# geoeo/ORB_SLAM3_V1.0

Measured on AMD Instinct MI355X. Metric: frames/sec ORB extract+match, 752x480 8-level 1000-feat; bit-exact kp/desc, higher is better.
Workload: dtype u8

## Files before the change

### orb_slam3_v1.0_amd/csrc/fast_common.h

```cpp
#pragma once
#include <hip/hip_runtime.h>
#include <stdint.h>

namespace orbfe {

constexpr int kFastTW = 64, kFastTH = 32;

constexpr int kFusedPyramidMinFrames = 0;

__device__ __forceinline__ bool arc9(uint32_t m)
{
    uint32_t m2 = m | (m << 16);
    uint32_t r = m2 & (m2 >> 1);
    r &= r >> 2;
    r &= r >> 4;
    r &= m2 >> 8;
    return (r & 0xffffu) != 0;
}

__device__ __forceinline__ bool corner_at_global(const uint8_t* __restrict__ img, int pitch, int x, int y, int th)
{
    const int8_t dy[16] = {3, 3, 2, 1, 0, -1, -2, -3, -3, -3, -2, -1, 0, 1, 2, 3};
    const int8_t dx[16] = {0, 1, 2, 3, 3, 3, 2, 1, 0, -1, -2, -3, -3, -3, -2, -1};
    const int v = img[(size_t)y * pitch + x];
    uint32_t mb = 0, md = 0;
#pragma unroll
    for (int k = 0; k < 16; k++) {
        const int d = (int)img[(size_t)(y + dy[k]) * pitch + x + dx[k]] - v;
        mb |= (uint32_t)(d > th) << k;
        md |= (uint32_t)(d < -th) << k;
    }
    return arc9(mb) || arc9(md);
}

}
```

### orb_slam3_v1.0_amd/csrc/kernels_quadtree.hip

```cpp
#include "launch.h"
#include "fast_common.h"

namespace orbfe {

constexpr int kQtThreads = 512;
constexpr int kQtThreadsSmall = 1024;
constexpr int kQtMaxRounds = 48;
constexpr uint32_t kKeyInf = 0x01000000u;

struct Box {
    int16_t ulx, urx, uly, bry;
};

__device__ __forceinline__ int child_code(const Box& b, int x, int y)
{
    const int halfX = (b.urx - b.ulx + 1) >> 1;
    const int halfY = (b.bry - b.uly + 1) >> 1;
    const int right = !(x < b.ulx + halfX);
    const int bottom = !(y < b.uly + halfY);
    return right + 2 * bottom;
}

__device__ __forceinline__ Box child_box(const Box& b, int c)
{
    const int halfX = (b.urx - b.ulx + 1) >> 1;
    const int halfY = (b.bry - b.uly + 1) >> 1;
    Box r;
    r.ulx = (c & 1) ? (int16_t)(b.ulx + halfX) : b.ulx;
    r.urx = (c & 1) ? b.urx : (int16_t)(b.ulx + halfX);
    r.uly = (c & 2) ? (int16_t)(b.uly + halfY) : b.uly;
    r.bry = (c & 2) ? b.bry : (int16_t)(b.uly + halfY);
    return r;
}

template <int NT>
__device__ __forceinline__ int block_excl_scan(int v, int& total, int* sWave)
{
    const int lane = threadIdx.x & 63, wave = threadIdx.x >> 6;
    int incl = v;
    incl += __builtin_amdgcn_update_dpp(0, incl, 0x111, 0xF, 0xF, true);
    incl += __builtin_amdgcn_update_dpp(0, incl, 0x112, 0xF, 0xF, true);
    incl += __builtin_amdgcn_update_dpp(0, incl, 0x114, 0xF, 0xF, true);
    incl += __builtin_amdgcn_update_dpp(0, incl, 0x118, 0xF, 0xF, true);
    incl += __builtin_amdgcn_update_dpp(0, incl, 0x142, 0xA, 0xF, true);
    incl += __builtin_amdgcn_update_dpp(0, incl, 0x143, 0xC, 0xF, true);
    __syncthreads();
    if (lane == 63) sWave[wave] = incl;
    __syncthreads();
    int base = 0, tot = 0;
#pragma unroll
    for (int i = 0; i < NT / 64; i++) {
        const int s = sWave[i];
        if (i < wave) base += s;
        tot += s;
    }
    total = tot;
    return base + incl - v;
}

template <int NT>
__device__ uint32_t pre_nms_cut_key(const PipelineDesc* __restrict__ P, const LevelDesc& L, int f, int l, bool high,
                                    int nFast, const uint8_t* __restrict__ gray0, size_t gray0FrameStride, int gray0Pitch,
                                    const uint8_t* __restrict__ ws, const uint16_t* __restrict__ tileRows, int* sWave,
                                    int* sRed)
{
    const int tid = threadIdx.x;
    const uint16_t* tr = tileRows + ((size_t)f * P->totalTiles + L.tileBase) * kFastTH;
    if (tid == 0) { sRed[0] = -1; sRed[1] = 0; sRed[2] = -1; }
    __syncthreads();
    int carry = 0;
    for (int base = 0; base < L.h; base += NT) {
        const int y = base + tid;
        int c = 0;
        if (y < L.h) {
            const int ty = y / kFastTH, r = y % kFastTH;
            for (int tx = 0; tx < L.tilesX; tx++) {
                const uint32_t v = tr[(size_t)(ty * L.tilesX + tx) * kFastTH + r];
                c += high ? (int)(v >> 8) : (int)(v & 0xffu);
            }
        }
        int tot;
        const int ex = block_excl_scan<NT>(c, tot, sWave) + carry;
        if (c > 0 && ex < nFast && ex + c >= nFast) { sRed[0] = y; sRed[1] = nFast - ex; }
        carry += tot;
        __syncthreads();
        if (sRed[0] >= 0) break;
    }
    const int ys = sRed[0], q = sRed[1];
    if (ys < 0) return kKeyInf;
    const uint8_t* img;
    int pitch;
    if (l == 0) {
        img = gray0 + (size_t)f * gray0FrameStride;
        pitch = gray0Pitch;
    } else {
        img = ws + L.imgOff + (size_t)f * L.imgFrameStride;
        pitch = L.pitch;
    }
    const int th = high ? P->iniTh : P->minTh;
    carry = 0;
    for (int base = 0; base < L.w; base += NT) {
        const int x = base + tid;
        int flag = 0;
        if (x > kEdge && x < L.w - kEdge) flag = corner_at_global(img, pitch, x, ys, th) ? 1 : 0;
        int tot;
        const int ex = block_excl_scan<NT>(flag, tot, sWave) + carry;
        if (flag && ex + 1 == q) sRed[2] = x;
        carry += tot;
        __syncthreads();
        if (sRed[2] >= 0) break;
    }
    const int xs = sRed[2];
    __syncthreads();
    if (xs < 0) return kKeyInf;
    return (((uint32_t)ys << kCoordBits) | (uint32_t)xs) + 1u;
}

__host__ __device__ constexpr size_t qt_scratch_bytes(int nc) { return (size_t)nc * (8 + 8 + 8 + 4 + 4 + 16 + 4 + 4 + 4 + 1 + 1); }

template <int NC, bool GLOBAL, int NT = kQtThreads>
__global__ __launch_bounds__(NT) __attribute__((amdgpu_waves_per_eu(NC <= 512 ? 8 : 1))) void quadtree_kernel(const PipelineDesc* __restrict__ P,
                                                             const uint32_t* __restrict__ cand,
                                                             uint16_t* __restrict__ nodeOfAll,
                                                             uint32_t* __restrict__ counters,
                                                             uint32_t* __restrict__ lvlKp,
                                                             const uint8_t* __restrict__ gray0, size_t gray0FrameStride,
                                                             int gray0Pitch, const uint8_t* __restrict__ ws,
                                                             const uint16_t* __restrict__ tileRows,
                                                             uint8_t* __restrict__ scratch)
{
    constexpr int IPT = NC / NT;
    static_assert(NC % NT == 0, "NC must be a multiple of the block size");

    Box* sBox[2];
    int* sCnt[2];
    int* sCC;
    int* sKeep;
    int* sS;
    uint8_t* sSplit;
    uint8_t* sNch;
    unsigned long long* sKey;
    int* sProc;
    if constexpr (!GLOBAL) {
        __shared__ Box lBox[2][NC];
        __shared__ int lCnt[2][NC];
        __shared__ int lCC[NC * 4];
        __shared__ int lKeep[NC];
        __shared__ int lS[NC];
        __shared__ uint8_t lSplit[NC];
        __shared__ uint8_t lNch[NC];
        __shared__ unsigned long long lKey[NC];
        __shared__ int lProc[NC];
        sBox[0] = lBox[0]; sBox[1] = lBox[1]; sCnt[0] = lCnt[0]; sCnt[1] = lCnt[1];
        sCC = lCC; sKeep = lKeep; sS = lS; sSplit = lSplit; sNch = lNch; sKey = lKey; sProc = lProc;
    } else {
        uint8_t* base = scratch + ((size_t)blockIdx.y * gridDim.x + blockIdx.x) * qt_scratch_bytes(NC);
        sKey = reinterpret_cast<unsigned long long*>(base); base += (size_t)NC * 8;
        sBox[0] = reinterpret_cast<Box*>(base); base += (size_t)NC * 8;
        sBox[1] = reinterpret_cast<Box*>(base); base += (size_t)NC * 8;
        sCnt[0] = reinterpret_cast<int*>(base); base += (size_t)NC * 4;
        sCnt[1] = reinterpret_cast<int*>(base); base += (size_t)NC * 4;
        sCC = reinterpret_cast<int*>(base); base += (size_t)NC * 16;
        sKeep = reinterpret_cast<int*>(base); base += (size_t)NC * 4;
        sS = reinterpret_cast<int*>(base); base += (size_t)NC * 4;
        sProc = reinterpret_cast<int*>(base); base += (size_t)NC * 4;
        sSplit = base; base += NC;
        sNch = base;
    }
    __shared__ int sWave[NT / 64];
    __shared__ int sRed[4];

    const int f = blockIdx.x, l = blockIdx.y;
    const int nL = P->nLevels;
    const LevelDesc& L = P->lv[l];
    const int tid = threadIdx.x;
    uint32_t* cnt = counters + ((size_t)f * nL + l) * kCntWords;
    const uint32_t* C = cand + L.candOff + (size_t)f * L.candCap;
    uint16_t* nodeOf = nodeOfAll + L.candOff + (size_t)f * L.candCap;
    uint32_t* out = lvlKp + (size_t)f * P->kpCapFrame + L.kpBase;

    const int N = L.nFeatures;
    const int nFast = P->nFast;
    const int iniTh = P->iniTh;
    const int nAll = (int)min(cnt[kCntCand], (uint32_t)L.candCap);
    uint32_t cutHi = kKeyInf, cutLo = kKeyInf;
    int cH = (int)cnt[kCntHigh];
    if ((int)cnt[kCntPreHigh] > nFast) {
        cutHi = pre_nms_cut_key<NT>(P, L, f, l, true, nFast, gray0, gray0FrameStride, gray0Pitch, ws, tileRows, sWave, sRed);
        int c = 0;
        for (int p = tid; p < nAll; p += NT) c += cand_score(C[p]) >= iniTh && cand_key(C[p]) < cutHi;
        block_excl_scan<NT>(c, cH, sWave);
    }
    const unsigned diff = (unsigned)nFast - (unsigned)cH;
    const bool retry = (double)diff > 0.25 * (double)nFast;
    int cL = nAll;
    if (retry && (int)cnt[kCntPreLow] > nFast) {
        cutLo = pre_nms_cut_key<NT>(P, L, f, l, false, nFast, gray0, gray0FrameStride, gray0Pitch, ws, tileRows, sWave, sRed);
        int c = 0;
        for (int p = tid; p < nAll; p += NT) c += cand_key(C[p]) < cutLo;
        block_excl_scan<NT>(c, cL, sWave);
    }
    uint32_t keyCut = cutLo;
    int lowKept = 0;
    if (retry && cL > 0) {
        lowKept = cL;
        if (cH + cL > nFast) lowKept = max(nFast - cH, 0);
    }
    if (retry && lowKept < cL) {
        uint32_t lo = 0, hi = kKeyInf;
        while (lo < hi) {
            const uint32_t mid = lo + ((hi - lo) >> 1);
            int c = 0;
            for (int p = tid; p < nAll; p += NT) c += cand_key(C[p]) < mid;
            int tot;
            block_excl_scan<NT>(c, tot, sWave);
            if (tot >= lowKept) hi = mid; else lo = mid + 1;
        }
        keyCut = min(lo, cutLo);
    }
    cL = nAll;
    const int totalPts = cH + lowKept;
    if (totalPts == 0) {
        if (tid == 0) cnt[kCntKp] = 0;
        return;
    }
    if (L.nodeCap > NC) {
        if (tid == 0) { cnt[kCntKp] = 0; atomicOr(&cnt[kCntStatus], (uint32_t)kFlagNodeOverflow); }
        return;
    }

#define PT_WEIGHT(cw) ((int)(cand_score(cw) >= iniTh && cand_key(cw) < cutHi) + (int)(retry && cand_key(cw) < keyCut))

    const int nIni = L.nIni;
    const float hX = L.hX;
    for (int i = tid; i < NC; i += NT) sCnt[0][i] = 0;
    __syncthreads();
    for (int p = tid; p < cL; p += NT) {
        const uint32_t cw = C[p];
        const int wgt = PT_WEIGHT(cw);
        if (wgt) atomicAdd(&sCnt[0][(int)((float)cand_x(cw) / hX)], wgt);
    }
    __syncthreads();
    if (tid == 0) {
        int n = 0;
        for (int i = 0; i < nIni; i++) {
            const int c = sCnt[0][i];
            sKeep[i] = n;
            if (c > 0) {
                Box b;
                b.ulx = (int16_t)(int)(hX * (float)i);
                b.urx = (int16_t)(int)(hX * (float)(i + 1));
                b.uly = 0;
                b.bry = (int16_t)L.h;
                sBox[1][n] = b;
                sCnt[1][n] = c;
                n++;
            }
        }
        sRed[0] = n;
    }
    __syncthreads();
    int n = sRed[0];
    for (int p = tid; p < cL; p += NT) {
        const uint32_t cw = C[p];
        if (PT_WEIGHT(cw)) nodeOf[p] = (uint16_t)sKeep[(int)((float)cand_x(cw) / hX)];
    }
    int cur = 1;
    bool sortedMode = false;
    bool overflow = false;

    for (int round = 0; round < kQtMaxRounds; round++) {
        const int prevSize = n;
        Box* box = cur ? sBox[1] : sBox[0];
        int* ncnt = cur ? sCnt[1] : sCnt[0];
        Box* nbox = cur ? sBox[0] : sBox[1];
        int* nncnt = cur ? sCnt[0] : sCnt[1];

        for (int i = tid; i < n * 4; i += NT) sCC[i] = 0;
        __syncthreads();
        for (int p0 = tid; p0 < cL; p0 += 4 * NT) {
            uint32_t cw4[4];
            int nd4[4];
#pragma unroll
            for (int k = 0; k < 4; k++) {
                const int p = p0 + k * NT;
                cw4[k] = p < cL ? C[p] : 0u;
                nd4[k] = p < cL ? (int)nodeOf[p] : 0;
            }
#pragma unroll
            for (int k = 0; k < 4; k++) {
                const uint32_t cw = cw4[k];
                const int wgt = (p0 + k * NT < cL) ? PT_WEIGHT(cw) : 0;
                if (wgt) {
                    const int i = nd4[k];
                    if (ncnt[i] > 1) atomicAdd(&sCC[4 * i + child_code(box[i], cand_x(cw), cand_y(cw))], wgt);
                }
            }
        }
        __syncthreads();

        int myExp[IPT], myNch[IPT];
#pragma unroll
        for (int k = 0; k < IPT; k++) {
            const int i = tid * IPT + k;
            int e = 0, nc = 0;
            if (i < n && ncnt[i] > 1) {
                e = 1;
                nc = (sCC[4 * i] > 0) + (sCC[4 * i + 1] > 0) + (sCC[4 * i + 2] > 0) + (sCC[4 * i + 3] > 0);
            }
            myExp[k] = e;
            myNch[k] = nc;
            if (i < NC) { sNch[i] = (uint8_t)nc; sSplit[i] = 0; }
        }

        int T = 0;
        if (!sortedMode) {
            int loc = 0;
#pragma unroll
            for (int k = 0; k < IPT; k++) loc += myNch[k];
            int base = block_excl_scan<NT>(loc, T, sWave);
#pragma unroll
            for (int k = 0; k < IPT; k++) {
                const int i = tid * IPT + k;
                if (i < n) {
                    sS[i] = base;
                    sSplit[i] = (uint8_t)myExp[k];
                }
                base += myNch[k];
            }
        } else {
#pragma unroll
            for (int k = 0; k < IPT; k++) {
                const int i = tid * IPT + k;
                if (i < n) {
                    unsigned long long key = 0;
                    if (myExp[k])
                        key = ((unsigned long long)(uint32_t)ncnt[i] << 40) |
                              ((unsigned long long)(uint16_t)box[i].ulx << 28) |
                              ((unsigned long long)(uint16_t)box[i].uly << 16) |
                              (unsigned long long)(0xFFFFu - (uint32_t)i);
                    sKey[i] = key;
                }
            }
            __syncthreads();
            int locM = 0;
#pragma unroll
            for (int k = 0; k < IPT; k++) locM += myExp[k];
            int m;
            block_excl_scan<NT>(locM, m, sWave);
#pragma unroll
            for (int k = 0; k < IPT; k++) {
                const int i = tid * IPT + k;
                if (i < n && myExp[k]) {
                    const unsigned long long key = sKey[i];
                    int r = 0;
                    for (int j = 0; j < n; j++) r += sKey[j] > key;
                    sProc[r] = i;
                }
            }
            __syncthreads();
            int locInc[IPT], locSum = 0;
#pragma unroll
            for (int k = 0; k < IPT; k++) {
                const int r = tid * IPT + k;
                locInc[k] = (r < m) ? (int)sNch[sProc[r]] - 1 : 0;
                locSum += locInc[k];
            }
            int totInc;
            int run = block_excl_scan<NT>(locSum, totInc, sWave);
            int myJ = m;
#pragma unroll
            for (int k = 0; k < IPT; k++) {
                const int r = tid * IPT + k;
                run += locInc[k];
                if (r < m && n + run >= N && myJ == m) myJ = r + 1;
            }
            if (tid == 0) sRed[1] = m;
            __syncthreads();
            if (myJ < m) atomicMin(&sRed[1], myJ);
            __syncthreads();
            const int J = sRed[1];
            int locN[IPT], locT = 0;
#pragma unroll
            for (int k = 0; k < IPT; k++) {
                const int r = tid * IPT + k;
                locN[k] = (r < J) ? (int)sNch[sProc[r]] : 0;
                locT += locN[k];
            }
            int base = block_excl_scan<NT>(locT, T, sWave);
#pragma unroll
            for (int k = 0; k < IPT; k++) {
                const int r = tid * IPT + k;
                if (r < J) {
                    const int i = sProc[r];
                    sS[i] = base;
                    sSplit[i] = 1;
                }
                base += locN[k];
            }
        }
        __syncthreads();

        int locK = 0;
#pragma unroll
        for (int k = 0; k < IPT; k++) {
            const int i = tid * IPT + k;
            locK += (i < n && !sSplit[i]) ? 1 : 0;
        }
        int K;
        int kbase = block_excl_scan<NT>(locK, K, sWave);
        const int newSize = T + K;
        if (newSize > NC) overflow = true;
        if (overflow) break;
        if (tid == 0) sRed[2] = 0;
        __syncthreads();

        int locExpand = 0;
#pragma unroll
        for (int k = 0; k < IPT; k++) {
            const int i = tid * IPT + k;
            if (i < n) {
                if (sSplit[i]) {
                    const Box b = box[i];
                    int kk = 0;
                    const int s = sS[i];
#pragma unroll
                    for (int c = 0; c < 4; c++) {
                        const int cc = sCC[4 * i + c];
                        if (cc > 0) {
                            const int pos = T - 1 - (s + kk);
                            nbox[pos] = child_box(b, c);
                            nncnt[pos] = cc;
                            sCC[4 * i + c] = pos;
                            locExpand += cc > 1;
                            kk++;
                        }
                    }
                } else {
                    const int pos = T + kbase;
                    nbox[pos] = box[i];
                    nncnt[pos] = ncnt[i];
                    sKeep[i] = pos;
                    kbase++;
                }
            }
        }
        if (locExpand) atomicAdd(&sRed[2], locExpand);
        __syncthreads();
        const int nToExpand = sRed[2];

        for (int p0 = tid; p0 < cL; p0 += 4 * NT) {
            uint32_t cw4[4];
            int nd4[4];
#pragma unroll
            for (int k = 0; k < 4; k++) {
                const int p = p0 + k * NT;
                cw4[k] = p < cL ? C[p] : 0u;
                nd4[k] = p < cL ? (int)nodeOf[p] : 0;
            }
#pragma unroll
            for (int k = 0; k < 4; k++) {
                const int p = p0 + k * NT;
                const uint32_t cw = cw4[k];
                if (p < cL && PT_WEIGHT(cw)) {
                    const int i = nd4[k];
                    nodeOf[p] = (uint16_t)(sSplit[i] ? sCC[4 * i + child_code(box[i], cand_x(cw), cand_y(cw))] : sKeep[i]);
                }
            }
        }
        __syncthreads();
        n = newSize;
        cur ^= 1;

        if (n >= N || n == prevSize) break;
        if (!sortedMode && n + 3 * nToExpand > N) sortedMode = true;
        if (round == kQtMaxRounds - 1 && tid == 0) atomicOr(&cnt[kCntStatus], (uint32_t)kFlagRoundLimit);
    }

    if (overflow) {
        if (tid == 0) { cnt[kCntKp] = 0; atomicOr(&cnt[kCntStatus], (uint32_t)kFlagNodeOverflow); }
        return;
    }

    int* bestResp = sCC;
    uint32_t* bestKey = reinterpret_cast<uint32_t*>(sCC + NC);
    for (int i = tid; i < n; i += NT) { bestResp[i] = 0; bestKey[i] = 0xFFFFFFFFu; }
    __syncthreads();
    for (int p = tid; p < cL; p += NT) {
        const uint32_t cw = C[p];
        if (PT_WEIGHT(cw)) atomicMax(&bestResp[nodeOf[p]], cand_score(cw));
    }
    __syncthreads();
    for (int p = tid; p < cL; p += NT) {
        const uint32_t cw = C[p];
        if (PT_WEIGHT(cw)) {
            const int i = nodeOf[p];
            if (cand_score(cw) == bestResp[i]) atomicMin(&bestKey[i], cand_key(cw));
        }
    }
    __syncthreads();
    for (int i = tid; i < n; i += NT) out[i] = ((uint32_t)bestResp[i] << 24) | bestKey[i];
    if (tid == 0) cnt[kCntKp] = (uint32_t)n;
#undef PT_WEIGHT
}

int quadtree_node_capacity(int maxNodeCap)
{
    const int caps[] = {512, 2048, 8192, 32768, 65536};
    for (int c : caps)
        if (maxNodeCap <= c && maxNodeCap <= 65535) return c;
    return 0;
}

size_t quadtree_scratch_bytes_per_block(int maxNodeCap)
{
    const int nc = quadtree_node_capacity(maxNodeCap);
    return nc > 2048 ? qt_scratch_bytes(nc) : 0;
}

void launch_quadtree(hipStream_t s, int frames, int nLevels, int maxNodeCap, const PipelineDesc* dP,
                     const uint32_t* cand, uint16_t* nodeOf, uint32_t* counters, uint32_t* lvlKp,
                     const uint8_t* gray0, size_t gray0FrameStride, int gray0Pitch, const uint8_t* ws,
                     const uint16_t* tileRows, uint8_t* scratch)
{
    dim3 grid(frames, nLevels);
    if ((long long)frames * nLevels <= 64 && quadtree_node_capacity(maxNodeCap) <= 2048) {
        dim3 blockS(kQtThreadsSmall);
        if (quadtree_node_capacity(maxNodeCap) <= 1024)
            hipLaunchKernelGGL((quadtree_kernel<1024, false, kQtThreadsSmall>), grid, blockS, 0, s, dP, cand, nodeOf, counters, lvlKp, gray0,
                               gray0FrameStride, gray0Pitch, ws, tileRows, scratch);
        else
            hipLaunchKernelGGL((quadtree_kernel<2048, false, kQtThreadsSmall>), grid, blockS, 0, s, dP, cand, nodeOf, counters, lvlKp, gray0,
                               gray0FrameStride, gray0Pitch, ws, tileRows, scratch);
        return;
    }
    dim3 block(kQtThreads);
#define ORBFE_QT(NCV, GLB)                                                                                        \
    hipLaunchKernelGGL((quadtree_kernel<NCV, GLB>), grid, block, 0, s, dP, cand, nodeOf, counters, lvlKp, gray0, \
                       gray0FrameStride, gray0Pitch, ws, tileRows, scratch)
    switch (quadtree_node_capacity(maxNodeCap)) {
    case 512: ORBFE_QT(512, false); break;
    case 2048: ORBFE_QT(2048, false); break;
    case 8192: ORBFE_QT(8192, true); break;
    case 32768: ORBFE_QT(32768, true); break;
    default: ORBFE_QT(65536, true); break;
    }
#undef ORBFE_QT
}

}
```

Measured before the change: 227,800.

## Keep quadtree candidates register-resident and fuse child counting into relabel pass

When a level has at most 4096 candidates and the kernel uses shared memory, the quadtree kernel now loads each candidate word and its node label into registers once and reuses them across every distribution round. The separate per-round child-count pass is folded into the previous round's relabel pass, which uses double-buffered child-count arrays so the global C/nodeOf reads drop out. Scans get double-buffered wave slots so a barrier can be dropped, two scans are fused into one, the sorted-mode rank loop runs only over compacted expandable keys with 16-byte loads, and the best-response selection becomes a single atomicMax on a packed key. This adds register pressure and doubles the child-count storage, which could lower occupancy.

```diff
diff --git a/orb_slam3_v1.0_amd/csrc/fast_common.h b/orb_slam3_v1.0_amd/csrc/fast_common.h
--- a/orb_slam3_v1.0_amd/csrc/fast_common.h
+++ b/orb_slam3_v1.0_amd/csrc/fast_common.h
@@ -7,6 +7,8 @@
 constexpr int kFastTW = 64, kFastTH = 32;
 
 constexpr int kFusedPyramidMinFrames = 0;
+
+constexpr int kQtResidentCap = 4096;
 
 __device__ __forceinline__ bool arc9(uint32_t m)
 {
diff --git a/orb_slam3_v1.0_amd/csrc/kernels_quadtree.hip b/orb_slam3_v1.0_amd/csrc/kernels_quadtree.hip
--- a/orb_slam3_v1.0_amd/csrc/kernels_quadtree.hip
+++ b/orb_slam3_v1.0_amd/csrc/kernels_quadtree.hip
@@ -33,10 +33,8 @@
     return r;
 }
 
-template <int NT>
-__device__ __forceinline__ int block_excl_scan(int v, int& total, int* sWave)
-{
-    const int lane = threadIdx.x & 63, wave = threadIdx.x >> 6;
+__device__ __forceinline__ int wave_incl_scan(int v)
+{
     int incl = v;
     incl += __builtin_amdgcn_update_dpp(0, incl, 0x111, 0xF, 0xF, true);
     incl += __builtin_amdgcn_update_dpp(0, incl, 0x112, 0xF, 0xF, true);
@@ -44,25 +42,62 @@
     incl += __builtin_amdgcn_update_dpp(0, incl, 0x118, 0xF, 0xF, true);
     incl += __builtin_amdgcn_update_dpp(0, incl, 0x142, 0xA, 0xF, true);
     incl += __builtin_amdgcn_update_dpp(0, incl, 0x143, 0xC, 0xF, true);
-    __syncthreads();
-    if (lane == 63) sWave[wave] = incl;
+    return incl;
+}
+
+template <int NT>
+__host__ __device__ constexpr int qt_wave_words() { return 2 * 2 * (NT / 64); }
+
+template <int NT>
+__device__ __forceinline__ int block_excl_scan(int v, int& total, int* sWave, int& par)
+{
+    constexpr int NW = NT / 64;
+    const int lane = threadIdx.x & 63, wave = threadIdx.x >> 6;
+    const int incl = wave_incl_scan(v);
+    int* w = sWave + par * 2 * NW;
+    par ^= 1;
+    if (lane == 63) w[wave] = incl;
     __syncthreads();
     int base = 0, tot = 0;
 #pragma unroll
-    for (int i = 0; i < NT / 64; i++) {
-        const int s = sWave[i];
+    for (int i = 0; i < NW; i++) {
+        const int s = w[i];
         if (i < wave) base += s;
         tot += s;
     }
-    total = tot;
+    total = __builtin_amdgcn_readfirstlane(tot);
     return base + incl - v;
+}
+
+template <int NT>
+__device__ __forceinline__ int block_excl_scan2(int a, int b, int& totA, int& totB, int& exB, int* sWave, int& par)
+{
+    constexpr int NW = NT / 64;
+    const int lane = threadIdx.x & 63, wave = threadIdx.x >> 6;
+    const int inA = wave_incl_scan(a), inB = wave_incl_scan(b);
+    int* w = sWave + par * 2 * NW;
+    par ^= 1;
+    if (lane == 63) { w[wave] = inA; w[NW + wave] = inB; }
+    __syncthreads();
+    int baseA = 0, tA = 0, baseB = 0, tB = 0;
+#pragma unroll
+    for (int i = 0; i < NW; i++) {
+        const int sa = w[i], sb = w[NW + i];
+        if (i < wave) { baseA += sa; baseB += sb; }
+        tA += sa;
+        tB += sb;
+    }
+    totA = __builtin_amdgcn_readfirstlane(tA);
+    totB = __builtin_amdgcn_readfirstlane(tB);
+    exB = baseB + inB - b;
+    return baseA + inA - a;
 }
 
 template <int NT>
 __device__ uint32_t pre_nms_cut_key(const PipelineDesc* __restrict__ P, const LevelDesc& L, int f, int l, bool high,
                                     int nFast, const uint8_t* __restrict__ gray0, size_t gray0FrameStride, int gray0Pitch,
                                     const uint8_t* __restrict__ ws, const uint16_t* __restrict__ tileRows, int* sWave,
-                                    int* sRed)
+                                    int& par, int* sRed)
 {
     const int tid = threadIdx.x;
     const uint16_t* tr = tileRows + ((size_t)f * P->totalTiles + L.tileBase) * kFastTH;
@@ -80,13 +115,13 @@
             }
         }
         int tot;
-        const int ex = block_excl_scan<NT>(c, tot, sWave) + carry;
+        const int ex = block_excl_scan<NT>(c, tot, sWave, par) + carry;
         if (c > 0 && ex < nFast && ex + c >= nFast) { sRed[0] = y; sRed[1] = nFast - ex; }
         carry += tot;
         __syncthreads();
         if (sRed[0] >= 0) break;
     }
-    const int ys = sRed[0], q = sRed[1];
+    const int ys = __builtin_amdgcn_readfirstlane(sRed[0]), q = __builtin_amdgcn_readfirstlane(sRed[1]);
     if (ys < 0) return kKeyInf;
     const uint8_t* img;
     int pitch;
@@ -104,19 +139,19 @@
         int flag = 0;
         if (x > kEdge && x < L.w - kEdge) flag = corner_at_global(img, pitch, x, ys, th) ? 1 : 0;
         int tot;
-        const int ex = block_excl_scan<NT>(flag, tot, sWave) + carry;
+        const int ex = block_excl_scan<NT>(flag, tot, sWave, par) + carry;
         if (flag && ex + 1 == q) sRed[2] = x;
         carry += tot;
         __syncthreads();
         if (sRed[2] >= 0) break;
     }
-    const int xs = sRed[2];
+    const int xs = __builtin_amdgcn_readfirstlane(sRed[2]);
     __syncthreads();
     if (xs < 0) return kKeyInf;
     return (((uint32_t)ys << kCoordBits) | (uint32_t)xs) + 1u;
 }
 
-__host__ __device__ constexpr size_t qt_scratch_bytes(int nc) { return (size_t)nc * (8 + 8 + 8 + 4 + 4 + 16 + 4 + 4 + 4 + 1 + 1); }
+__host__ __device__ constexpr size_t qt_scratch_bytes(int nc) { return (size_t)nc * (8 + 8 + 8 + 4 + 4 + 16 + 16 + 4 + 4 + 4 + 1 + 1); }
 
 template <int NC, bool GLOBAL, int NT = kQtThreads>
 __global__ __launch_bounds__(NT) __attribute__((amdgpu_waves_per_eu(NC <= 512 ? 8 : 1))) void quadtree_kernel(const PipelineDesc* __restrict__ P,
@@ -134,7 +169,7 @@
 
     Box* sBox[2];
     int* sCnt[2];
-    int* sCC;
+    int* sCCt[2];
     int* sKeep;
     int* sS;
     uint8_t* sSplit;
@@ -144,15 +179,15 @@
     if constexpr (!GLOBAL) {
         __shared__ Box lBox[2][NC];
         __shared__ int lCnt[2][NC];
-        __shared__ int lCC[NC * 4];
+        __shared__ __attribute__((aligned(16))) int lCC[2][NC * 4];
         __shared__ int lKeep[NC];
         __shared__ int lS[NC];
         __shared__ uint8_t lSplit[NC];
         __shared__ uint8_t lNch[NC];
-        __shared__ unsigned long long lKey[NC];
+        __shared__ __attribute__((aligned(16))) unsigned long long lKey[NC];
         __shared__ int lProc[NC];
         sBox[0] = lBox[0]; sBox[1] = lBox[1]; sCnt[0] = lCnt[0]; sCnt[1] = lCnt[1];
-        sCC = lCC; sKeep = lKeep; sS = lS; sSplit = lSplit; sNch = lNch; sKey = lKey; sProc = lProc;
+        sCCt[0] = lCC[0]; sCCt[1] = lCC[1]; sKeep = lKeep; sS = lS; sSplit = lSplit; sNch = lNch; sKey = lKey; sProc = lProc;
     } else {
         uint8_t* base = scratch + ((size_t)blockIdx.y * gridDim.x + blockIdx.x) * qt_scratch_bytes(NC);
         sKey = reinterpret_cast<unsigned long long*>(base); base += (size_t)NC * 8;
@@ -160,15 +195,17 @@
         sBox[1] = reinterpret_cast<Box*>(base); base += (size_t)NC * 8;
         sCnt[0] = reinterpret_cast<int*>(base); base += (size_t)NC * 4;
         sCnt[1] = reinterpret_cast<int*>(base); base += (size_t)NC * 4;
-        sCC = reinterpret_cast<int*>(base); base += (size_t)NC * 16;
+        sCCt[0] = reinterpret_cast<int*>(base); base += (size_t)NC * 16;
+        sCCt[1] = reinterpret_cast<int*>(base); base += (size_t)NC * 16;
         sKeep = reinterpret_cast<int*>(base); base += (size_t)NC * 4;
         sS = reinterpret_cast<int*>(base); base += (size_t)NC * 4;
         sProc = reinterpret_cast<int*>(base); base += (size_t)NC * 4;
         sSplit = base; base += NC;
         sNch = base;
     }
-    __shared__ int sWave[NT / 64];
+    __shared__ int sWave[qt_wave_words<NT>()];
     __shared__ int sRed[4];
+    int par = 0;
 
     const int f = blockIdx.x, l = blockIdx.y;
     const int nL = P->nLevels;
@@ -183,22 +220,34 @@
     const int nFast = P->nFast;
     const int iniTh = P->iniTh;
     const int nAll = (int)min(cnt[kCntCand], (uint32_t)L.candCap);
+    constexpr int KREG = GLOBAL ? 1 : kQtResidentCap / NT;
+    static_assert(GLOBAL || KREG * NT == kQtResidentCap, "the block size must divide kQtResidentCap");
+    const bool resident = !GLOBAL && nAll <= kQtResidentCap;
+    uint32_t rcw[KREG];
+    int rst[KREG];
+    if (resident) {
+#pragma unroll
+        for (int k = 0; k < KREG; k++) {
+            const int p = tid + k * NT;
+            rcw[k] = p < nAll ? C[p] : 0u;
+        }
+    }
     uint32_t cutHi = kKeyInf, cutLo = kKeyInf;
     int cH = (int)cnt[kCntHigh];
     if ((int)cnt[kCntPreHigh] > nFast) {
-        cutHi = pre_nms_cut_key<NT>(P, L, f, l, true, nFast, gray0, gray0FrameStride, gray0Pitch, ws, tileRows, sWave, sRed);
+        cutHi = pre_nms_cut_key<NT>(P, L, f, l, true, nFast, gray0, gray0FrameStride, gray0Pitch, ws, tileRows, sWave, par, sRed);
         int c = 0;
         for (int p = tid; p < nAll; p += NT) c += cand_score(C[p]) >= iniTh && cand_key(C[p]) < cutHi;
-        block_excl_scan<NT>(c, cH, sWave);
+        block_excl_scan<NT>(c, cH, sWave, par);
     }
     const unsigned diff = (unsigned)nFast - (unsigned)cH;
     const bool retry = (double)diff > 0.25 * (double)nFast;
     int cL = nAll;
     if (retry && (int)cnt[kCntPreLow] > nFast) {
-        cutLo = pre_nms_cut_key<NT>(P, L, f, l, false, nFast, gray0, gray0FrameStride, gray0Pitch, ws, tileRows, sWave, sRed);
+        cutLo = pre_nms_cut_key<NT>(P, L, f, l, false, nFast, gray0, gray0FrameStride, gray0Pitch, ws, tileRows, sWave, par, sRed);
         int c = 0;
         for (int p = tid; p < nAll; p += NT) c += cand_key(C[p]) < cutLo;
-        block_excl_scan<NT>(c, cL, sWave);
+        block_excl_scan<NT>(c, cL, sWave, par);
     }
     uint32_t keyCut = cutLo;
     int lowKept = 0;
@@ -213,7 +262,7 @@
             int c = 0;
             for (int p = tid; p < nAll; p += NT) c += cand_key(C[p]) < mid;
             int tot;
-            block_excl_scan<NT>(c, tot, sWave);
+            block_excl_scan<NT>(c, tot, sWave, par);
             if (tot >= lowKept) hi = mid; else lo = mid + 1;
         }
         keyCut = min(lo, cutLo);
@@ -231,15 +280,57 @@
 
 #define PT_WEIGHT(cw) ((int)(cand_score(cw) >= iniTh && cand_key(cw) < cutHi) + (int)(retry && cand_key(cw) < keyCut))
 
+    if (resident) {
+#pragma unroll
+        for (int k = 0; k < KREG; k++) rst[k] = (tid + k * NT < nAll) ? PT_WEIGHT(rcw[k]) << 16 : 0;
+    }
+    auto cand_pass = [&](auto readLabel, auto writeLabel, auto&& f) {
+        constexpr bool READ = decltype(readLabel)::value, WRITE = decltype(writeLabel)::value;
+        if (resident) {
+#pragma unroll
+            for (int k = 0; k < KREG; k++) {
+                const int st = rst[k], wgt = st >> 16;
+                asm volatile("" : "+v"(rcw[k]));
+                if (wgt) {
+                    const int lab = f(rcw[k], wgt, st & 0xFFFF);
+                    if constexpr (WRITE) rst[k] = (wgt << 16) | lab;
+                }
+            }
+            return;
+        }
+        for (int p0 = tid; p0 < cL; p0 += 4 * NT) {
+            uint32_t cw4[4];
+            int nd4[4];
+#pragma unroll
+            for (int k = 0; k < 4; k++) {
+                const int p = p0 + k * NT;
+                cw4[k] = p < cL ? C[p] : 0u;
+                nd4[k] = (READ && p < cL) ? (int)nodeOf[p] : 0;
+            }
+#pragma unroll
+            for (int k = 0; k < 4; k++) {
+                const int p = p0 + k * NT;
+                const uint32_t cw = cw4[k];
+                const int wgt = p < cL ? PT_WEIGHT(cw) : 0;
+                if (wgt) {
+                    const int lab = f(cw, wgt, nd4[k]);
+                    if constexpr (WRITE) nodeOf[p] = (uint16_t)lab;
+                }
+            }
+        }
+    };
+    constexpr std::true_type yes{};
+    constexpr std::false_type no{};
+
     const int nIni = L.nIni;
     const float hX = L.hX;
     for (int i = tid; i < NC; i += NT) sCnt[0][i] = 0;
-    __syncthreads();
-    for (int p = tid; p < cL; p += NT) {
-        const uint32_t cw = C[p];
-        const int wgt = PT_WEIGHT(cw);
-        if (wgt) atomicAdd(&sCnt[0][(int)((float)cand_x(cw) / hX)], wgt);
-    }
+    for (int i = tid; i < 4 * nIni; i += NT) sCCt[1][i] = 0;
+    __syncthreads();
+    cand_pass(no, no, [&](uint32_t cw, int wgt, int) {
+        atomicAdd(&sCnt[0][(int)((float)cand_x(cw) / hX)], wgt);
+        return 0;
+    });
     __syncthreads();
     if (tid == 0) {
         int n = 0;
@@ -260,11 +351,13 @@
         sRed[0] = n;
     }
     __syncthreads();
-    int n = sRed[0];
-    for (int p = tid; p < cL; p += NT) {
-        const uint32_t cw = C[p];
-        if (PT_WEIGHT(cw)) nodeOf[p] = (uint16_t)sKeep[(int)((float)cand_x(cw) / hX)];
-    }
+    int n = __builtin_amdgcn_readfirstlane(sRed[0]);
+    cand_pass(no, yes, [&](uint32_t cw, int wgt, int) {
+        const int i = sKeep[(int)((float)cand_x(cw) / hX)];
+        if (sCnt[1][i] > 1) atomicAdd(&sCCt[1][4 * i + child_code(sBox[1][i], cand_x(cw), cand_y(cw))], wgt);
+        return i;
+    });
+    __syncthreads();
     int cur = 1;
     bool sortedMode = false;
     bool overflow = false;
@@ -275,29 +368,10 @@
         int* ncnt = cur ? sCnt[1] : sCnt[0];
         Box* nbox = cur ? sBox[0] : sBox[1];
         int* nncnt = cur ? sCnt[0] : sCnt[1];
-
-        for (int i = tid; i < n * 4; i += NT) sCC[i] = 0;
-        __syncthreads();
-        for (int p0 = tid; p0 < cL; p0 += 4 * NT) {
-            uint32_t cw4[4];
-            int nd4[4];
-#pragma unroll
-            for (int k = 0; k < 4; k++) {
-                const int p = p0 + k * NT;
-                cw4[k] = p < cL ? C[p] : 0u;
-                nd4[k] = p < cL ? (int)nodeOf[p] : 0;
-            }
-#pragma unroll
-            for (int k = 0; k < 4; k++) {
-                const uint32_t cw = cw4[k];
-                const int wgt = (p0 + k * NT < cL) ? PT_WEIGHT(cw) : 0;
-                if (wgt) {
-                    const int i = nd4[k];
-                    if (ncnt[i] > 1) atomicAdd(&sCC[4 * i + child_code(box[i], cand_x(cw), cand_y(cw))], wgt);
-                }
-            }
-        }
-        __syncthreads();
+        int* sCC = cur ? sCCt[1] : sCCt[0];
+        int* nCC = cur ? sCCt[0] : sCCt[1];
+
+        if (tid == 0) sRed[2] = 0;
 
         int myExp[IPT], myNch[IPT];
 #pragma unroll
@@ -310,15 +384,18 @@
             }
             myExp[k] = e;
             myNch[k] = nc;
-            if (i < NC) { sNch[i] = (uint8_t)nc; sSplit[i] = 0; }
-        }
-
-        int T = 0;
+            if (i < NC) sNch[i] = (uint8_t)nc;
+        }
+
+        int T = 0, K = 0, kbase = 0;
         if (!sortedMode) {
-            int loc = 0;
-#pragma unroll
-            for (int k = 0; k < IPT; k++) loc += myNch[k];
-            int base = block_excl_scan<NT>(loc, T, sWave);
+            int locT = 0, locK = 0;
+#pragma unroll
+            for (int k = 0; k < IPT; k++) {
+                locT += myNch[k];
+                locK += (tid * IPT + k < n && !myExp[k]) ? 1 : 0;
+            }
+            int base = block_excl_scan2<NT>(locT, locK, T, K, kbase, sWave, par);
 #pragma unroll
             for (int k = 0; k < IPT; k++) {
                 const int i = tid * IPT + k;
@@ -329,33 +406,42 @@
                 base += myNch[k];
             }
         } else {
+            unsigned long long myKey[IPT];
+            int locM = 0;
 #pragma unroll
             for (int k = 0; k < IPT; k++) {
                 const int i = tid * IPT + k;
-                if (i < n) {
-                    unsigned long long key = 0;
-                    if (myExp[k])
-                        key = ((unsigned long long)(uint32_t)ncnt[i] << 40) |
-                              ((unsigned long long)(uint16_t)box[i].ulx << 28) |
-                              ((unsigned long long)(uint16_t)box[i].uly << 16) |
-                              (unsigned long long)(0xFFFFu - (uint32_t)i);
-                    sKey[i] = key;
-                }
+                myKey[k] = 0;
+                if (myExp[k])
+                    myKey[k] = ((unsigned long long)(uint32_t)ncnt[i] << 40) |
+                               ((unsigned long long)(uint16_t)box[i].ulx << 28) |
+                               ((unsigned long long)(uint16_t)box[i].uly << 16) |
+                               (unsigned long long)(0xFFFFu - (uint32_t)i);
+                locM += myExp[k];
+            }
+            int m;
+            int mpos = block_excl_scan<NT>(locM, m, sWave, par);
+#pragma unroll
+            for (int k = 0; k < IPT; k++)
+                if (myExp[k]) sKey[mpos++] = myKey[k];
+            if (tid == 0) {
+                if (m & 1) sKey[m] = 0;
+                sRed[1] = m;
             }
             __syncthreads();
-            int locM = 0;
-#pragma unroll
-            for (int k = 0; k < IPT; k++) locM += myExp[k];
-            int m;
-            block_excl_scan<NT>(locM, m, sWave);
-#pragma unroll
-            for (int k = 0; k < IPT; k++) {
-                const int i = tid * IPT + k;
-                if (i < n && myExp[k]) {
-                    const unsigned long long key = sKey[i];
+            int myRank[IPT];
+#pragma unroll
+            for (int k = 0; k < IPT; k++) {
+                myRank[k] = NC;
+                if (myExp[k]) {
+                    const unsigned long long key = myKey[k];
                     int r = 0;
-                    for (int j = 0; j < n; j++) r += sKey[j] > key;
-                    sProc[r] = i;
+                    for (int j = 0; j < m; j += 2) {
+                        const ulonglong2 kk = *reinterpret_cast<const ulonglong2*>(&sKey[j]);
+                        r += (int)(kk.x > key) + (int)(kk.y > key);
+                    }
+                    myRank[k] = r;
+                    sProc[r] = tid * IPT + k;
                 }
             }
             __syncthreads();
@@ -367,53 +453,38 @@
                 locSum += locInc[k];
             }
             int totInc;
-            int run = block_excl_scan<NT>(locSum, totInc, sWave);
-            int myJ = m;
+            int run = n + block_excl_scan<NT>(locSum, totInc, sWave, par);
 #pragma unroll
             for (int k = 0; k < IPT; k++) {
                 const int r = tid * IPT + k;
+                const int before = run;
                 run += locInc[k];
-                if (r < m && n + run >= N && myJ == m) myJ = r + 1;
-            }
-            if (tid == 0) sRed[1] = m;
+                if (r < m && before < N && run >= N) sRed[1] = r + 1;
+            }
             __syncthreads();
-            if (myJ < m) atomicMin(&sRed[1], myJ);
-            __syncthreads();
-            const int J = sRed[1];
-            int locN[IPT], locT = 0;
+            const int J = __builtin_amdgcn_readfirstlane(sRed[1]);
+            int locN[IPT], locT = 0, locK = 0;
 #pragma unroll
             for (int k = 0; k < IPT; k++) {
                 const int r = tid * IPT + k;
                 locN[k] = (r < J) ? (int)sNch[sProc[r]] : 0;
                 locT += locN[k];
-            }
-            int base = block_excl_scan<NT>(locT, T, sWave);
+                locK += (r < n && !(myRank[k] < J)) ? 1 : 0;
+            }
+            int base = block_excl_scan2<NT>(locT, locK, T, K, kbase, sWave, par);
 #pragma unroll
             for (int k = 0; k < IPT; k++) {
                 const int r = tid * IPT + k;
-                if (r < J) {
-                    const int i = sProc[r];
-                    sS[i] = base;
-                    sSplit[i] = 1;
-                }
+                if (r < J) sS[sProc[r]] = base;
                 base += locN[k];
-            }
-        }
-        __syncthreads();
-
-        int locK = 0;
-#pragma unroll
-        for (int k = 0; k < IPT; k++) {
-            const int i = tid * IPT + k;
-            locK += (i < n && !sSplit[i]) ? 1 : 0;
-        }
-        int K;
-        int kbase = block_excl_scan<NT>(locK, K, sWave);
+                if (r < n) sSplit[r] = (uint8_t)(myRank[k] < J);
+            }
+            __syncthreads();
+        }
         const int newSize = T + K;
         if (newSize > NC) overflow = true;
         if (overflow) break;
-        if (tid == 0) sRed[2] = 0;
-        __syncthreads();
+        const bool countNext = newSize < N && newSize != prevSize;
 
         int locExpand = 0;
 #pragma unroll
@@ -431,7 +502,8 @@
                             const int pos = T - 1 - (s + kk);
                             nbox[pos] = child_box(b, c);
                             nncnt[pos] = cc;
-                            sCC[4 * i + c] = pos;
+                            sCC[4 * i + c] = pos | ((cc > 1) << 16);
+                            if (countNext) *reinterpret_cast<int4*>(&nCC[4 * pos]) = make_int4(0, 0, 0, 0);
                             locExpand += cc > 1;
                             kk++;
                         }
@@ -440,34 +512,31 @@
                     const int pos = T + kbase;
                     nbox[pos] = box[i];
                     nncnt[pos] = ncnt[i];
-                    sKeep[i] = pos;
+                    sKeep[i] = pos | ((ncnt[i] > 1) << 16);
+                    if (countNext) *reinterpret_cast<int4*>(&nCC[4 * pos]) = make_int4(0, 0, 0, 0);
                     kbase++;
                 }
             }
         }
         if (locExpand) atomicAdd(&sRed[2], locExpand);
         __syncthreads();
-        const int nToExpand = sRed[2];
-
-        for (int p0 = tid; p0 < cL; p0 += 4 * NT) {
-            uint32_t cw4[4];
-            int nd4[4];
-#pragma unroll
-            for (int k = 0; k < 4; k++) {
-                const int p = p0 + k * NT;
-                cw4[k] = p < cL ? C[p] : 0u;
-                nd4[k] = p < cL ? (int)nodeOf[p] : 0;
-            }
-#pragma unroll
-            for (int k = 0; k < 4; k++) {
-                const int p = p0 + k * NT;
-                const uint32_t cw = cw4[k];
-                if (p < cL && PT_WEIGHT(cw)) {
-                    const int i = nd4[k];
-                    nodeOf[p] = (uint16_t)(sSplit[i] ? sCC[4 * i + child_code(box[i], cand_x(cw), cand_y(cw))] : sKeep[i]);
-                }
-            }
-        }
+        const int nToExpand = __builtin_amdgcn_readfirstlane(sRed[2]);
+
+        cand_pass(yes, yes, [&](uint32_t cw, int wgt, int i) {
+            const int x = cand_x(cw), y = cand_y(cw);
+            Box b = box[i];
+            int e;
+            if (sSplit[i]) {
+                const int c = child_code(b, x, y);
+                e = sCC[4 * i + c];
+                b = child_box(b, c);
+            } else {
+                e = sKeep[i];
+            }
+            const int pos = e & 0xFFFF;
+            if (countNext && (e >> 16)) atomicAdd(&nCC[4 * pos + child_code(b, x, y)], wgt);
+            return pos;
+        });
         __syncthreads();
         n = newSize;
         cur ^= 1;
@@ -482,24 +551,15 @@
         return;
     }
 
-    int* bestResp = sCC;
-    uint32_t* bestKey = reinterpret_cast<uint32_t*>(sCC + NC);
-    for (int i = tid; i < n; i += NT) { bestResp[i] = 0; bestKey[i] = 0xFFFFFFFFu; }
-    __syncthreads();
-    for (int p = tid; p < cL; p += NT) {
-        const uint32_t cw = C[p];
-        if (PT_WEIGHT(cw)) atomicMax(&bestResp[nodeOf[p]], cand_score(cw));
-    }
-    __syncthreads();
-    for (int p = tid; p < cL; p += NT) {
-        const uint32_t cw = C[p];
-        if (PT_WEIGHT(cw)) {
-            const int i = nodeOf[p];
-            if (cand_score(cw) == bestResp[i]) atomicMin(&bestKey[i], cand_key(cw));
-        }
-    }
-    __syncthreads();
-    for (int i = tid; i < n; i += NT) out[i] = ((uint32_t)bestResp[i] << 24) | bestKey[i];
+    uint32_t* best = reinterpret_cast<uint32_t*>(sCCt[0]);
+    for (int i = tid; i < n; i += NT) best[i] = 0u;
+    __syncthreads();
+    cand_pass(yes, no, [&](uint32_t cw, int, int i) {
+        atomicMax(&best[i], cw ^ 0x00FFFFFFu);
+        return i;
+    });
+    __syncthreads();
+    for (int i = tid; i < n; i += NT) out[i] = best[i] ^ 0x00FFFFFFu;
     if (tid == 0) cnt[kCntKp] = (uint32_t)n;
 #undef PT_WEIGHT
 }
```

Result: faster. 230,400, median of 6 (+1.1%).
